# bastienjossen/DDL25Spring

Hardware: AMD Instinct MI355X
Metric: FedAvg rounds/sec + local samples/sec, ResNet-18 CIFAR-10-shape, 8 clients (higher is better)
Workload: dtype fp32; 1 GPU; model=resnet18-cifar10, global_batch=800, parallelism=fedavg-8clients-dp1, clients=8, local_batch=100, local_epochs=1, samples_per_client=6250, client_slots_per_gpu=8, hip_graphs=True, fp32_conv_math=auto

## Files before the change

### csrc/kernels/conv_x6hw.hip

```cpp
#include <cstdlib>

#include "ddl_common.h"
#include "conv_f32_core.h"

namespace {

typedef float f16v __attribute__((ext_vector_type(16)));

constexpr int HW_BK = 64, HW_BC = 32, HW_TP = 128;
constexpr int HW_KS = 136;
constexpr unsigned HW_OOB = 0x80000000u;

struct HWGeo {
  int lgW;
  int SR;
  int NSEG;
  int HR, HCp;
  int CS;
  int ntile;
  int NUX;
  int probe;
};

typedef int hw_rsrc __attribute__((ext_vector_type(4)));
__device__ __forceinline__ hw_rsrc hw_make_rsrc(const void* p, long long bytes) {
  const unsigned long long a = (unsigned long long)p;
  hw_rsrc r;
  r.x = (int)(unsigned)(a & 0xffffffffull);
  r.y = (int)(unsigned)((a >> 32) & 0xffffull);
  r.z = (int)bytes;
  r.w = 0x00020000;
  return r;
}
__device__ __forceinline__ void hw_load(f4v& d, const hw_rsrc& rs, unsigned off) {
  asm volatile("buffer_load_dwordx4 %0, %1, %2, 0 offen" : "=a"(d) : "v"(off), "s"(rs) : "memory");
}

__device__ __forceinline__ void split8(const float (&v)[8], s8v& h, s8v& m, s8v& l) {
  s4v h0, m0, l0, h1, m1, l1;
  split3(make_float4(v[0], v[1], v[2], v[3]), h0, m0, l0);
  split3(make_float4(v[4], v[5], v[6], v[7]), h1, m1, l1);
  h = cat44(h0, h1);
  m = cat44(m0, m1);
  l = cat44(l0, l1);
}

template <int RS, int NUX>
__global__ __launch_bounds__(256, 1) void convx6hw_kernel(ConvF32Args a, HWGeo hg) {
  constexpr int T = RS * RS, PD = (RS - 1) / 2;
  extern __shared__ __attribute__((aligned(16))) char smem[];
  bf16_t* const dyl = (bf16_t*)smem;
  bf16_t* const xl = dyl + 3 * HW_BK * HW_KS;
  const int tid = threadIdx.x, lane = tid & 63, wid = tid >> 6;
  const int OW = 1 << hg.lgW, TR = HW_TP >> hg.lgW;
  const int nct = a.C / HW_BC;
  const int k0 = (blockIdx.x / nct) * HW_BK, c0 = (blockIdx.x % nct) * HW_BC;
  const int split = blockIdx.y, nsplit = gridDim.y, g = blockIdx.z;
  const int per = (hg.ntile + nsplit - 1) / nsplit;
  const int t0 = split * per, t1 = min(hg.ntile, t0 + per);
  const int K = a.K, C = a.C, H = a.H, W = a.W;
  const long long npix = (long long)a.N * H * W;

  const hw_rsrc rD = hw_make_rsrc(a.dy + (long long)g * a.dy_gs, npix * K * 4);
  const hw_rsrc rX = hw_make_rsrc(a.x + (long long)g * a.x_gs, npix * C * 4);

  const int dkc = tid & 15, dpg = tid >> 4;
  const int ncol8 = hg.HCp >> 3;
  const int nxu = 8 * hg.NSEG * hg.HR * ncol8;
  const bool xf = a.in_scale != nullptr;
  float4 xsc[NUX], xsh[NUX];
#pragma unroll
  for (int u = 0; u < NUX; ++u) {
    xsc[u] = make_float4(1.f, 1.f, 1.f, 1.f);
    xsh[u] = make_float4(0.f, 0.f, 0.f, 0.f);
    const int uu = tid + 256 * u;
    if (xf && uu < nxu) {
      const long long cc = (long long)g * C + c0 + 4 * (uu & 7);
      xsc[u] = *(const float4*)(a.in_scale + cc);
      xsh[u] = *(const float4*)(a.in_shift + cc);
    }
  }

  int useg[NUX], uhr[NUX], uxc[NUX], uoff[NUX];
  bool uvalid[NUX];
#pragma unroll
  for (int u = 0; u < NUX; ++u) {
    const int uu = tid + 256 * u, rest = uu >> 3;
    const int xc = rest % ncol8, xrr = rest / ncol8;
    useg[u] = xrr / hg.HR;
    uhr[u] = xrr - useg[u] * hg.HR;
    uxc[u] = xc;
    uoff[u] = 4 * (uu & 7) * hg.CS + xrr * hg.HCp + 8 * xc;
    uvalid[u] = uu < nxu;
  }
  f4v rd[8], rx[NUX][8];
  unsigned xok[NUX];
  auto load_tile = [&](int tile) {
#pragma unroll
    for (int j = 0; j < 8; ++j) {
      const int p = tile * HW_TP + dpg * 8 + j;
      hw_load(rd[j], rD, p < npix ? (unsigned)((p * K + k0 + 4 * dkc) * 4) : HW_OOB);
    }
    const int row0 = tile * TR;
    const int n0 = row0 / a.P, oh0 = row0 - n0 * a.P;
#pragma unroll
    for (int u = 0; u < NUX; ++u) {
      xok[u] = 0;
      const int n = n0 + useg[u];
      const int ih = oh0 + uhr[u] - PD;
#pragma unroll
      for (int j = 0; j < 8; ++j) {
        const int iw = 8 * uxc[u] + j - PD;
        const bool ok = uvalid[u] && n < a.N && (unsigned)ih < (unsigned)H && (unsigned)iw < (unsigned)W;
        xok[u] |= (ok ? 1u : 0u) << j;
        hw_load(rx[u][j], rX, ok ? (unsigned)((((n * H + ih) * W + iw) * C + c0 + 4 * (tid & 7)) * 4) : HW_OOB);
      }
    }
  };
  s8v sd[4][3], sx[NUX][4][3];
  auto hw_wait = [&]() {
    asm volatile("s_waitcnt vmcnt(0)" ::: "memory");
#pragma unroll
    for (int j = 0; j < 8; ++j) asm volatile("" : "+a"(rd[j]));
#pragma unroll
    for (int u = 0; u < NUX; ++u)
#pragma unroll
      for (int j = 0; j < 8; ++j) asm volatile("" : "+a"(rx[u][j]));
  };
  auto split_tile = [&]() {
#pragma unroll
    for (int ch = 0; ch < 4; ++ch) {
      float v[8];
#pragma unroll
      for (int j = 0; j < 8; ++j) v[j] = ch == 0 ? rd[j].x : ch == 1 ? rd[j].y : ch == 2 ? rd[j].z : rd[j].w;
      split8(v, sd[ch][0], sd[ch][1], sd[ch][2]);
    }
  };
  auto write_tile = [&]() {
#pragma unroll
    for (int ch = 0; ch < 4; ++ch) {
      bf16_t* d = dyl + (4 * dkc + ch) * HW_KS + 8 * dpg;
#pragma unroll
      for (int pl = 0; pl < 3; ++pl) *(s8v*)(d + pl * HW_BK * HW_KS) = sd[ch][pl];
    }
#pragma unroll
    for (int u = 0; u < NUX; ++u) {
#pragma unroll
      for (int ch = 0; ch < 4; ++ch) {
        const float sc = ch == 0 ? xsc[u].x : ch == 1 ? xsc[u].y : ch == 2 ? xsc[u].z : xsc[u].w;
        const float sh = ch == 0 ? xsh[u].x : ch == 1 ? xsh[u].y : ch == 2 ? xsh[u].z : xsh[u].w;
        float v[8];
#pragma unroll
        for (int j = 0; j < 8; ++j) {
          float e = ch == 0 ? rx[u][j].x : ch == 1 ? rx[u][j].y : ch == 2 ? rx[u][j].z : rx[u][j].w;
          if (xf && ((xok[u] >> j) & 1u)) {
            e = e * sc + sh;
            if (a.in_relu) e = fmaxf(e, 0.f);
          }
          v[j] = e;
        }
        split8(v, sx[u][ch][0], sx[u][ch][1], sx[u][ch][2]);
      }
    }
#pragma unroll
    for (int u = 0; u < NUX; ++u) {
      if (!uvalid[u]) continue;
#pragma unroll
      for (int ch = 0; ch < 4; ++ch) {
        bf16_t* d = xl + uoff[u] + ch * hg.CS;
#pragma unroll
        for (int pl = 0; pl < 3; ++pl) *(s8v*)(d + pl * HW_BC * hg.CS) = sx[u][ch][pl];
      }
    }
  };

  const int kb = wid >> 1, kh = wid & 1;
  const int arow = (kb * 32 + (lane & 31)) * HW_KS;
  auto xbase = [&](int ks) {
    const int p = 16 * ks + 8 * (lane >> 5);
    const int prow = p >> hg.lgW, pcol = p & (OW - 1);
    const int seg = prow / hg.SR, r = prow - seg * hg.SR;
    return (lane & 31) * hg.CS + (seg * hg.HR + r) * hg.HCp + pcol;
  };
  f16v acc[T];
#pragma unroll
  for (int t = 0; t < T; ++t)
#pragma unroll
    for (int v = 0; v < 16; ++v) acc[t][v] = 0.f;

  if (t0 < t1) {
    if (!(hg.probe & 4)) load_tile(t0);
    for (int tile = t0; tile < t1; ++tile) {
      __syncthreads();
      hw_wait();
      if (!(hg.probe & 1)) {
        split_tile();
        write_tile();
      }
      if (tile + 1 < t1 && !(hg.probe & 4)) load_tile(tile + 1);
      __syncthreads();
      if (hg.probe & 2) continue;
#pragma unroll 1
      for (int ip = 0; ip < 2; ++ip) {
        s8v ah[2], am[2], al[2];
        int xb[2];
#pragma unroll
        for (int j = 0; j < 2; ++j) {
          const int ks = 4 * ip + 2 * j + kh;
          xb[j] = xbase(ks);
          const bf16_t* ap = dyl + arow + 16 * ks + 8 * (lane >> 5);
          ah[j] = *(const s8v*)ap;
          am[j] = *(const s8v*)(ap + HW_BK * HW_KS);
          al[j] = *(const s8v*)(ap + 2 * HW_BK * HW_KS);
        }
#pragma unroll
        for (int r = 0; r < RS; ++r) {
          f16v c[RS];
#pragma unroll
          for (int j = 0; j < 2; ++j) {
            const bf16_t* bp = xl + xb[j] + r * hg.HCp;
            s8v bh[RS], bm[RS], bl[RS];
            const s8v h0 = *(const s8v*)bp, m0 = *(const s8v*)(bp + HW_BC * hg.CS),
                      l0 = *(const s8v*)(bp + 2 * HW_BC * hg.CS);
            bh[0] = h0; bm[0] = m0; bl[0] = l0;
            if constexpr (RS == 3) {
              const s8v h1 = *(const s8v*)(bp + 8), m1 = *(const s8v*)(bp + 8 + HW_BC * hg.CS),
                        l1 = *(const s8v*)(bp + 8 + 2 * HW_BC * hg.CS);
              bh[1] = __builtin_shufflevector(h0, h1, 1, 2, 3, 4, 5, 6, 7, 8);
              bm[1] = __builtin_shufflevector(m0, m1, 1, 2, 3, 4, 5, 6, 7, 8);
              bl[1] = __builtin_shufflevector(l0, l1, 1, 2, 3, 4, 5, 6, 7, 8);
              bh[2] = __builtin_shufflevector(h0, h1, 2, 3, 4, 5, 6, 7, 8, 9);
              bm[2] = __builtin_shufflevector(m0, m1, 2, 3, 4, 5, 6, 7, 8, 9);
              bl[2] = __builtin_shufflevector(l0, l1, 2, 3, 4, 5, 6, 7, 8, 9);
            }
#pragma unroll
            for (int s2 = 0; s2 < RS; ++s2)
              c[s2] = __builtin_amdgcn_mfma_f32_32x32x16_bf16(al[j], bh[s2], j ? c[s2] : (f16v){}, 0, 0, 0);
#pragma unroll
            for (int s2 = 0; s2 < RS; ++s2) c[s2] = __builtin_amdgcn_mfma_f32_32x32x16_bf16(ah[j], bl[s2], c[s2], 0, 0, 0);
#pragma unroll
            for (int s2 = 0; s2 < RS; ++s2) c[s2] = __builtin_amdgcn_mfma_f32_32x32x16_bf16(am[j], bm[s2], c[s2], 0, 0, 0);
#pragma unroll
            for (int s2 = 0; s2 < RS; ++s2) c[s2] = __builtin_amdgcn_mfma_f32_32x32x16_bf16(ah[j], bm[s2], c[s2], 0, 0, 0);
#pragma unroll
            for (int s2 = 0; s2 < RS; ++s2) c[s2] = __builtin_amdgcn_mfma_f32_32x32x16_bf16(am[j], bh[s2], c[s2], 0, 0, 0);
#pragma unroll
            for (int s2 = 0; s2 < RS; ++s2) c[s2] = __builtin_amdgcn_mfma_f32_32x32x16_bf16(ah[j], bh[s2], c[s2], 0, 0, 0);
          }
#pragma unroll
          for (int s2 = 0; s2 < RS; ++s2) {
#pragma unroll
            for (int v = 0; v < 16; ++v) acc[r * RS + s2][v] = acc[r * RS + s2][v] + c[s2][v];
          }
        }
      }
    }
  }

  __syncthreads();
  float* const red = (float*)smem;
  if (kh == 1) {
#pragma unroll
    for (int t = 0; t < T; ++t)
#pragma unroll
      for (int v = 0; v < 16; ++v) red[((kb * T + t) * 16 + v) * 64 + lane] = acc[t][v];
  }
  __syncthreads();
  if (kh == 1) return;
#pragma unroll
  for (int t = 0; t < T; ++t)
#pragma unroll
    for (int v = 0; v < 16; ++v) acc[t][v] = acc[t][v] + red[((kb * T + t) * 16 + v) * 64 + lane];

  const long long qd = (long long)T * C;
  const bool split_store = nsplit > 1;
  float* dst = split_store ? a.partial + ((long long)split * a.G + g) * K * qd : a.out + (long long)g * a.out_gs;
#pragma unroll
  for (int t = 0; t < T; ++t) {
    float old[16];
#pragma unroll
    for (int v = 0; v < 16; ++v) {
      const int k = k0 + kb * 32 + 8 * (v >> 2) + 4 * (lane >> 5) + (v & 3);
      const long long off = (long long)k * qd + (long long)t * C + c0 + (lane & 31);
      old[v] = (!split_store && a.accumulate) ? dst[off] : 0.f;
    }
#pragma unroll
    for (int v = 0; v < 16; ++v) {
      const int k = k0 + kb * 32 + 8 * (v >> 2) + 4 * (lane >> 5) + (v & 3);
      const long long off = (long long)k * qd + (long long)t * C + c0 + (lane & 31);
      dst[off] = split_store ? acc[t][v] : old[v] + a.gscale * acc[t][v];
    }
  }
}

}

static bool hw_geo(const ConvF32Args& a, HWGeo& h, int& rs) {
  if (a.stride != 1 || a.R != a.S || (a.R != 1 && a.R != 3) || a.pad != (a.R - 1) / 2) return false;
  if (a.P != a.H || a.Q != a.W || a.K % HW_BK || a.C % HW_BC) return false;
  const int OW = a.Q, OH = a.P;
  if (OW < 8 || OW > HW_TP || (OW & (OW - 1))) return false;
  rs = a.R;
  int lg = 0;
  while ((1 << lg) < OW) ++lg;
  const int TR = HW_TP / OW;
  int SR;
  if (TR <= OH) {
    if (OH % TR) return false;
    SR = TR;
  } else {
    if (TR % OH) return false;
    SR = OH;
  }
  h.lgW = lg;
  h.SR = SR;
  h.NSEG = TR / SR;
  h.HR = SR + a.R - 1;
  h.HCp = (OW + a.S - 1 + 7) / 8 * 8;
  const int img = h.NSEG * h.HR * h.HCp;
  h.CS = (img - 8 + 127) / 128 * 128 + 8;
  const long long npix = (long long)a.N * a.P * a.Q;
  h.ntile = (int)((npix + HW_TP - 1) / HW_TP);
  const int nxu = 8 * h.NSEG * h.HR * (h.HCp / 8);
  h.NUX = (nxu + 255) / 256;
  if (h.NUX > 2) return false;
  static const int probe = getenv("DDL_HW_PROBE") ? atoi(getenv("DDL_HW_PROBE")) : 0;
  h.probe = probe;
  const long long lim = (1LL << 31) - 64;
  if (npix * a.C * 4 > lim || npix * a.K * 4 > lim) return false;
  return true;
}

static size_t hw_lds(const HWGeo& h, int T) {
  const size_t stage = (size_t)3 * (HW_BK * HW_KS + HW_BC * h.CS) * 2;
  const size_t red = (size_t)2 * T * 16 * 64 * 4;
  return stage > red ? stage : red;
}

extern "C" __attribute__((visibility("default"))) int ddl_x6hw_ok(const ConvF32Args* ap) {
  HWGeo h;
  int rs;
  return hw_geo(*ap, h, rs) && hw_lds(h, rs * rs) <= 160 * 1024 ? 1 : 0;
}

extern "C" __attribute__((visibility("default"))) int ddl_x6hw_tiles(const ConvF32Args* ap) {
  HWGeo h;
  int rs;
  return hw_geo(*ap, h, rs) ? h.ntile : 0;
}

template <int RS, int NUX>
static int launch_hw(const ConvF32Args& a, const HWGeo& h, hipStream_t s) {
  const int split = a.split_k < 1 ? 1 : a.split_k;
  const size_t lds = hw_lds(h, RS * RS);
  static bool attr_set = false;
  if (!attr_set) {
    hipFuncSetAttribute((const void*)convx6hw_kernel<RS, NUX>, hipFuncAttributeMaxDynamicSharedMemorySize,
                        160 * 1024);
    attr_set = true;
  }
  const dim3 grid((unsigned)((a.K / HW_BK) * (a.C / HW_BC)), (unsigned)split, (unsigned)a.G);
  hipLaunchKernelGGL((convx6hw_kernel<RS, NUX>), grid, dim3(256), lds, s, a, h);
  return (int)hipGetLastError();
}

extern "C" __attribute__((visibility("default"))) int ddl_x6hw(const ConvF32Args* ap, hipStream_t s) {
  const ConvF32Args& a = *ap;
  HWGeo h;
  int rs;
  if (a.G < 1 || a.N < 1 || !hw_geo(a, h, rs) || hw_lds(h, rs * rs) > 160 * 1024) return (int)hipErrorInvalidValue;
  const int split = a.split_k < 1 ? 1 : a.split_k;
  if (split > 1) {
    const long long need = (long long)split * a.G * a.K * a.R * a.S * a.C;
    if (!a.partial || need > a.partial_cap) return (int)hipErrorInvalidValue;
  }
  int e;
  if (rs == 3) e = h.NUX == 1 ? launch_hw<3, 1>(a, h, s) : launch_hw<3, 2>(a, h, s);
  else e = h.NUX == 1 ? launch_hw<1, 1>(a, h, s) : launch_hw<1, 2>(a, h, s);
  return e;
}
```

### ddl25spring_amd/ops/functional_f32.py

```python
from __future__ import annotations

import ctypes
import math
import os

import torch

from . import _lib
from . import workspace as ws
from ._lib import check, ptr, stream

F_FWD, F_DGRAD, F_WGRAD = 0, 1, 2
WS_CAP = 1 << 26
_WS: dict = {}
TARGET_WG = int(os.environ.get("DDL_F32_TARGET_WG", "640"))


def is_f32(t) -> bool:
    return t is not None and t.is_cuda and t.dtype == torch.float32


class SlotStats:
    __slots__ = ("t", "rows")

# ... 377 lines not shown
    def __exit__(self, *exc):
        _PRESPLIT[0] = self._prev
        if self._pending is not None:
            torch.cuda.current_stream().wait_event(self._pending)
            self._pending = None
        if self.state == "record" and self.keys and not torch.cuda.is_current_stream_capturing() \
                and exc[0] is None:
            self._build()
        return False

    def _build(self):
        lib = _lib.kernels()
        if lib.ddl_x6_split_desc_size() != ctypes.sizeof(_SplitDesc):
            raise RuntimeError("ABI mismatch for SplitDesc")
        dev = torch.device("cuda", torch.cuda.current_device())
        vol = [k[2] * k[3] * k[4] * k[5] for k in self.keys]
        nhead = len(self.keys)
        if PRESPLIT_SIDE[0] and len(self.keys) > 1:
            nhead, acc = 1, vol[0]
            while nhead < len(self.keys) and acc + vol[nhead] <= PRESPLIT_HEAD_FRAC * sum(vol):
                acc += vol[nhead]
                nhead += 1
        self.tail = set(self.keys[nhead:])
        self.tables = []
        for part in (self.keys[:nhead], self.keys[nhead:]):
            if not part:
                continue
            descs = (_SplitDesc * len(part))()
            blk = 0
            for i, key in enumerate(part):
                w, layout, G, K, T, C, w_gs = key
                buf = torch.empty(G, K * T * C * 6, dtype=torch.uint8, device=dev)
                self.bufs[key] = buf
                nblk = max(1, min(1024, -(-G * K * T * C // 16 // 256)))
                d = descs[i]
                d.w, d.out, d.w_gs, d.o_gs = w, buf.data_ptr(), w_gs, buf.stride(0)
                d.G, d.K, d.T, d.C, d.layout, d.blk0, d.nblk = G, K, T, C, layout, blk, nblk
                blk += nblk
            raw = torch.frombuffer(bytearray(bytes(descs)), dtype=torch.uint8)
            self.tables.append((raw.to(dev), len(part), blk))
        self.state = "ready"


def _store_identity(owner):
    store = getattr(owner, "store", None)
    data = getattr(store, "data", None)
    if data is None:
        return None
    return data.data_ptr(), data.numel(), id(data.untyped_storage())


def presplit_scope(owner) -> "PresplitScope | contextlib.nullcontext":
    sig = _store_identity(owner)
    sc = getattr(owner, "_f32_presplit", None)
    if sc is None or getattr(owner, "_f32_presplit_sig", None) != sig:
        sc = PresplitScope()
        owner._f32_presplit = sc
        owner._f32_presplit_sig = sig
    return sc


def _slots(a, mode: int, geom) -> int:
    cfg, _ = plan(mode, geom)
    if uses_halo(mode, geom):
        return int(_lib.kernels().ddl_x6h_slots(ctypes.byref(a), mode))
    return int(_lib.kernels().ddl_convf32_slots(ctypes.byref(a), mode, _cfg(cfg)))


def slot_rows(mode: int, geom) -> int:
    cfg, _ = plan(mode, geom)
    bq = ((_cfg(cfg) >> 8) & 0xFF) * 16
    if uses_halo(mode, geom) and geom.Q & (geom.Q - 1):
        return bq // (1 << (geom.Q - 1).bit_length()) * geom.Q
    return bq


def _xform(in_bn):
    if in_bn is None:
        return {}
    sc, sh = in_bn
    assert sc.is_contiguous() and sh.is_contiguous()
    return dict(in_scale=ptr(sc), in_shift=ptr(sh), in_relu=1)


def conv_fwd(x, w, geom, bias=None, relu=False, stats=None, out=None, residual=None, in_bn=None, split_k=0):
    y = out if out is not None else torch.empty(geom.G, geom.N, geom.P, geom.Q, geom.K, dtype=torch.float32,
                                                device=x.device)
    if residual is not None and (residual.stride(0) != y.stride(0) or not residual.is_contiguous()):
        residual = residual.contiguous()
    geom = _launch_geom(geom, "f")
    a = _args(geom, x=ptr(x), w=ptr(w), out=ptr(y), bias=ptr(bias), residual=ptr(residual),
              x_gs=_gs(x), w_gs=_gs(w), out_gs=_gs(y), bias_gs=_gs(bias), relu=int(bool(relu)), **_xform(in_bn))
    if stats is not None:
        st = torch.empty(geom.G, _slots(a, F_FWD, geom), 2, geom.K, dtype=torch.float32, device=x.device)
        a.stats = ptr(st)
        if isinstance(stats, SlotStats):
            stats.t = st
            stats.rows = slot_rows(F_FWD, geom)
        else:
            raise TypeError("fp32 conv statistics go to a SlotStats (Fn.stats_buffer(..., like=x))")
    _launch(a, F_FWD, geom, x.device, split_k)
    return y


def conv_dgrad(dy, w, geom, residual=None, mask=None, out=None, bn=None, mask_bn=None, residual_sub=1,
               split_k=0, dy_bn=None, dy_bn_out=None):
    dx = out if out is not None else torch.empty(geom.G, geom.N, geom.H, geom.W, geom.C, dtype=torch.float32,
                                                 device=dy.device)
    if residual_sub == 1:
        geom = _launch_geom(geom, "d")
    kw = {}
    if dy_bn is not None:
        xb, coef = dy_bn
        assert xb.is_contiguous() and coef.is_contiguous() and xb.shape == dy.shape and dy.is_contiguous()
        if uses_halo(F_DGRAD, geom) and split_k == 0:
            kw.update(dyb_x=ptr(xb), dyb_coef=ptr(coef), dyb_out=ptr(dy_bn_out))
        else:
            dy = coef_apply(dy, xb, coef, out=dy_bn_out)
    if residual is not None and residual_sub == 2 and geom.H & 1 and uses_halo(F_DGRAD, geom) \
            and (split_k or plan(F_DGRAD, geom)[1]) <= 1:
        full = torch.zeros_like(dx)
        full[:, :, ::2, ::2] = residual
        residual, residual_sub = full, 1
    if residual is not None:
        if residual_sub == 2:
            want = (geom.G, geom.N, (geom.H + 1) // 2, (geom.W + 1) // 2, geom.C)
            assert tuple(residual.shape) == want, (tuple(residual.shape), want)
            residual = residual.contiguous()
            kw.update(res_sub=2, res_gs=residual.stride(0))
        elif residual.stride(0) != dx.stride(0) or not residual.is_contiguous():
            residual = residual.contiguous()
    if mask is not None and (mask.stride(0) != dx.stride(0) or not mask.is_contiguous()):
        mask = mask.contiguous()
    if bn is not None:
        x, mean, rstd = bn
        assert x.is_contiguous() and x.stride(0) == dx.stride(0) and mean.is_contiguous() and rstd.is_contiguous()
        kw.update(bn_x=ptr(x), bn_mean=ptr(mean), bn_rstd=ptr(rstd))
        if mask_bn is not None:
            sc, sh = mask_bn
            assert sc.is_contiguous() and sh.is_contiguous() and sc.numel() == geom.G * geom.C
            kw.update(mask_scale=ptr(sc), mask_shift=ptr(sh))
    a = _args(geom, w=ptr(w), dy=ptr(dy), out=ptr(dx), residual=ptr(residual), mask=ptr(mask),
              w_gs=_gs(w), dy_gs=_gs(dy), out_gs=_gs(dx), **kw)
    part = None
    if bn is not None:
        part = torch.empty(geom.G, _slots(a, F_DGRAD, geom), 2, geom.C, dtype=torch.float32, device=dy.device)
        a.stats = ptr(part)
    _launch(a, F_DGRAD, geom, dy.device, split_k)
    return dx if bn is None else (dx, part)


HALO_WGRAD = [os.environ.get("DDL_F32_HALO_WGRAD", "1") != "0"]
HW_MIN_W = int(os.environ.get("DDL_F32_HW_MIN_W", "16"))
HW_TARGET_WG = int(os.environ.get("DDL_F32_HW_TARGET_WG", "256"))


def uses_halo_wgrad(geom) -> bool:
    a = _args(geom)
    return HALO_WGRAD[0] and _MATH[0] != "mfma32" and geom.W >= HW_MIN_W \
        and bool(_lib.kernels().ddl_x6hw_ok(ctypes.byref(a)))


def _halo_wgrad(a, geom, device, split_k: int, ws_role: str) -> bool:
    if not (HALO_WGRAD[0] and _MATH[0] != "mfma32") or geom.W < HW_MIN_W \
            or not _lib.kernels().ddl_x6hw_ok(ctypes.byref(a)):
        return False
    lib = _lib.kernels()
    ntile = int(lib.ddl_x6hw_tiles(ctypes.byref(a)))
    base = (geom.K // 64) * (geom.C // 32) * geom.G
    split = split_k or 1
    if not split_k and TARGET_WG != 1:
        _tuned(F_WGRAD, geom)
        p = _TUNED.get(f"x6hw:wgrad:{geom.G},{geom.N},{geom.H},{geom.W},{geom.C},{geom.K},{geom.R},{geom.S},"
                       f"{geom.stride},{geom.pad}")
        if p is not None:
            split_k = split = int(p[0])
    if not split_k:
        target = min(HW_TARGET_WG, TARGET_WG)
        while base * split < target and ntile >= split * 2 * 3 and split < 128:
            split *= 2
    n = geom.K * geom.R * geom.S * geom.C
    if split > 1:
        buf = workspace(device, ws_role)
        while split > 1 and split * geom.G * n > buf.numel():
            split //= 2
        if split > 1:
            a.partial, a.partial_cap = buf.data_ptr(), buf.numel()
    a.split_k = split
    check(lib.ddl_x6hw(ctypes.byref(a), stream()), "conv_wgrad_f32_halo")
    if split > 1:
        check(lib.ddl_convf32_wgrad_reduce(a.partial, a.out, a.out_gs, geom.G, n, split, a.accumulate, a.gscale,
                                           stream()), "conv_wgrad_f32_halo_reduce")
    return True


def conv_wgrad(dy, x, geom, dw, accumulate=True, gscale=1.0, in_bn=None, split_k=0, ws_role="main"):
    if not accumulate and gscale != 1.0:
        raise ValueError("a scaled WGRAD must accumulate (it adds into the master weights)")
    geom = _launch_geom(geom, "w")
    a = _args(geom, x=ptr(x), dy=ptr(dy), out=ptr(dw), x_gs=_gs(x), dy_gs=_gs(dy), out_gs=_gs(dw),
              accumulate=int(bool(accumulate)), gscale=float(gscale), **_xform(in_bn))
    if (F_WGRAD, geom) not in _OVERRIDE and _halo_wgrad(a, geom, dy.device, split_k, ws_role):
        return dw
    _launch(a, F_WGRAD, geom, dy.device, split_k, ws_role)
    return dw


def _bnf_args(stats, gamma, beta, running_mean, running_var, count, eps, momentum, training, outs, G, C,
              tile_rows=0):
    a = _lib.BNFArgs()
    a.tile_rows = int(tile_rows)
    a.stats, a.gamma, a.beta = ptr(stats), ptr(gamma), ptr(beta)
    a.running_mean, a.running_var = ptr(running_mean), ptr(running_var)
    a.scale, a.shift, a.mean, a.rstd = (ptr(outs[i]) for i in range(4))
    a.gs_param = _gs(gamma) if gamma is not None else _gs(beta)
    a.gs_buf = _gs(running_mean)
    a.G, a.C, a.count = G, C, int(count)
    a.eps, a.momentum, a.training = float(eps), float(momentum), int(training)
    a.stripes = stats.shape[1] if stats is not None else 0
    return a


def bn_finalize_many(items, eps=1e-5, momentum=0.1, training=True):
    dev = items[0][1].device if items[0][1] is not None else items[0][3].device
    args, outs = [], []
    for stats, gamma, beta, rm, rv, count, G, C in items:
        t = stats.t if isinstance(stats, SlotStats) else stats
        rows = stats.rows if isinstance(stats, SlotStats) else 0
        if training:
            assert t is not None and t.is_contiguous(), "fp32 BN statistics missing (conv not run?)"
        o = torch.empty(4, G, C, dtype=torch.float32, device=dev)
        args.append(_bnf_args(t if training else None, gamma, beta, rm, rv, count, eps, momentum, training, o, G, C,
                              rows))
        outs.append(o)
    b = ctypes.byref(args[1]) if len(args) > 1 else None
    check(_lib.kernels().ddl_bnf_finalize(ctypes.byref(args[0]), b, stream()), "bn_finalize_f32")
    return [(o[0], o[1], o[2], o[3]) for o in outs]


def bn_apply(x, scale, shift, r=None, rscale=None, rshift=None, act=0, out=None):
    assert x.is_contiguous() and (r is None or r.is_contiguous())
    y = out if out is not None else torch.empty_like(x)
    G, C = x.shape[0], x.shape[-1]
    check(_lib.kernels().ddl_bnf_apply(ptr(x), ptr(scale), ptr(shift), ptr(r), ptr(rscale), ptr(rshift), ptr(y),
                                       x[0].numel(), C, G, act, stream()), "bn_apply_f32")
    return y


def reduce_slots(M: int, C: int, G: int) -> int:
    return int(_lib.kernels().ddl_bnf_reduce_slots(int(M), int(C), int(G)))


def bn_bwd_reduce_part(dy, ymask, x, mean, rstd):
    G, C = x.shape[0], x.shape[-1]
    M = x[0].numel() // C
    part = torch.empty(G, reduce_slots(M, C, G), 2, C, dtype=torch.float32, device=x.device)
    check(_lib.kernels().ddl_bnf_reduce(ptr(dy), ptr(ymask), ptr(x), ptr(mean), ptr(rstd), ptr(part), M, C, G,
                                        stream()), "bn_bwd_reduce_f32")
    return part


def bn_stats(x):
    G, C = x.shape[0], x.shape[-1]
    M = x[0].numel() // C
    st = SlotStats()
    st.t = torch.empty(G, reduce_slots(M, C, G), 2, C, dtype=torch.float32, device=x.device)
    check(_lib.kernels().ddl_bnf_stats(ptr(x), ptr(st.t), M, C, G, stream()), "bn_stats_f32")
    return st


def _bwd_args(x, mean, rstd, gamma, dgamma, dbeta, part, dx, fold_slots: int = 0, coef=None):
    G, C = x.shape[0], x.shape[-1]
    t = _lib.BNFBwdArgs()
    if coef is None:
        coef = ws.scratch_uninit((G, 3, C), x.device)
    gs = _gs(gamma) if gamma is not None else 0
    if dgamma is not None or dbeta is not None:
        gd = _gs(dgamma) if dgamma is not None else _gs(dbeta)
        assert gamma is None or gd == gs, "gamma and its gradient must share the group stride"
        gs = gd
    t.x, t.mean, t.rstd, t.gamma = ptr(x), ptr(mean), ptr(rstd), ptr(gamma)
    t.dgamma, t.dbeta, t.part, t.coef, t.dx, t.gs_param = ptr(dgamma), ptr(dbeta), ptr(part), ptr(coef), ptr(dx), gs
    t.slots = part.shape[1] if part is not None else 0
    S = max(fold_slots, t.slots)
    fws = None
    if FOLD2[0] and S > 0:
        fws = torch.empty(int(_lib.kernels().ddl_bnf_fold_ws(S, C, G)), dtype=torch.float64, device=x.device)
        t.fold_ws = fws.data_ptr()
        if FOLD1L[0] and x.is_cuda:
            t.tickets = _fold_tickets(x.device, int(_lib.kernels().ddl_bnf_fold_tickets(C, G)))
    t._keep = (coef, fws)
    return t


FOLD2 = [os.environ.get("DDL_F32_FOLD2", "1") != "0"]
FOLD1L = [os.environ.get("DDL_F32_FOLD1L", "1") != "0"]
_TICKETS: dict = {}


TICKETS_N = 1 << 16


def _dev_key(device) -> str:
    d = torch.device(device)
    return f"cuda:{d.index if d.index is not None else torch.cuda.current_device()}"


def _fold_tickets(device, n: int) -> int:
    key = _dev_key(device)
    buf = _TICKETS.get(key)
    if buf is None:
        if torch.cuda.is_current_stream_capturing():
            raise RuntimeError("fp32 BN fold counters first requested inside a graph capture: run one eager "
                               "step (or functional_f32.ensure_workspace) before capturing")
        buf = torch.zeros(TICKETS_N, dtype=torch.int32, device=device)
        _TICKETS[key] = buf
    if n > buf.numel():
        raise ValueError(f"BN fold needs {n} counters (> {buf.numel()})")
    return buf.data_ptr()


def fold_tickets_clean() -> bool:
    torch.cuda.synchronize()
    return all(int(b.abs().sum().item()) == 0 for b in _TICKETS.values())


def bn_backward(dy, ymask, x, mean, rstd, gamma, dgamma=None, dbeta=None, emit_dym=False, part=None):
    G, C = x.shape[0], x.shape[-1]
    M = x[0].numel() // C
    assert dy.is_contiguous() and x.is_contiguous()
    do_reduce = part is None
    if do_reduce:
# ... 115 lines not shown
```

Before: 38310 samples/s.

## Warp-specialize halo wgrad kernel with double-buffered LDS staging waves

Restructures the halo weight-gradient conv kernel into 512 threads, with four producer waves that load, split to bf16x3 and stage tiles into a double-buffered LDS region. Four consumer waves run the MFMA loops, so global loads and splitting overlap with matrix math instead of alternating with it. The pixel tile is halved to 64, and the split granularity is now counted in tile pairs. It also adds a W=4 variant, which the Python side only uses for small widths when a tuned entry exists. In exchange it doubles LDS usage, holds two register tile sets in the producers, and changes how split-K is sized.

Result: faster. 39270 samples/s (median of 6 runs) (+2.5%).

```diff
diff --git a/csrc/kernels/conv_x6hw.hip b/csrc/kernels/conv_x6hw.hip
--- a/csrc/kernels/conv_x6hw.hip
+++ b/csrc/kernels/conv_x6hw.hip
@@ -7,8 +7,10 @@
 
 typedef float f16v __attribute__((ext_vector_type(16)));
 
-constexpr int HW_BK = 64, HW_BC = 32, HW_TP = 128;
-constexpr int HW_KS = 136;
+constexpr int HW_BK = 64, HW_BC = 32, HW_TP = 64;
+constexpr int HW_KS = 72;
+constexpr int HW_NT = 512;
+constexpr size_t HW_LDS_MAX = 160 * 1024;
 constexpr unsigned HW_OOB = 0x80000000u;
 
 struct HWGeo {
@@ -18,7 +20,6 @@
   int HR, HCp;
   int CS;
   int ntile;
-  int NUX;
   int probe;
 };
 
@@ -33,7 +34,7 @@
   return r;
 }
 __device__ __forceinline__ void hw_load(f4v& d, const hw_rsrc& rs, unsigned off) {
-  asm volatile("buffer_load_dwordx4 %0, %1, %2, 0 offen" : "=a"(d) : "v"(off), "s"(rs) : "memory");
+  asm volatile("buffer_load_dwordx4 %0, %1, %2, 0 offen" : "=v"(d) : "v"(off), "s"(rs) : "memory");
 }
 
 __device__ __forceinline__ void split8(const float (&v)[8], s8v& h, s8v& m, s8v& l) {
@@ -45,18 +46,35 @@
   l = cat44(l0, l1);
 }
 
-template <int RS, int NUX>
-__global__ __launch_bounds__(256, 1) void convx6hw_kernel(ConvF32Args a, HWGeo hg) {
+template <bool W4>
+__device__ __forceinline__ s8v hw_win(const s8v& c0, const s8v& c1, int s) {
+  if constexpr (W4) {
+    if (s == 0) return __builtin_shufflevector(c0, c1, 0, 1, 2, 3, 8, 9, 10, 11);
+    if (s == 1) return __builtin_shufflevector(c0, c1, 1, 2, 3, 4, 9, 10, 11, 12);
+    return __builtin_shufflevector(c0, c1, 2, 3, 4, 5, 10, 11, 12, 13);
+  } else {
+    if (s == 0) return c0;
+    if (s == 1) return __builtin_shufflevector(c0, c1, 1, 2, 3, 4, 5, 6, 7, 8);
+    return __builtin_shufflevector(c0, c1, 2, 3, 4, 5, 6, 7, 8, 9);
+  }
+}
+
+template <int RS, bool W4>
+__global__ __launch_bounds__(HW_NT) void convx6hw_kernel(ConvF32Args a, HWGeo hg) {
   constexpr int T = RS * RS, PD = (RS - 1) / 2;
   extern __shared__ __attribute__((aligned(16))) char smem[];
+  const int stg = 3 * (HW_BK * HW_KS + HW_BC * hg.CS);
   bf16_t* const dyl = (bf16_t*)smem;
   bf16_t* const xl = dyl + 3 * HW_BK * HW_KS;
-  const int tid = threadIdx.x, lane = tid & 63, wid = tid >> 6;
+  const int tid = threadIdx.x, lane = tid & 63;
+  const int wid = __builtin_amdgcn_readfirstlane(tid >> 6);
+  const bool stager = wid < 4;
+  const int ptid = tid & 255;
   const int OW = 1 << hg.lgW, TR = HW_TP >> hg.lgW;
   const int nct = a.C / HW_BC;
   const int k0 = (blockIdx.x / nct) * HW_BK, c0 = (blockIdx.x % nct) * HW_BC;
   const int split = blockIdx.y, nsplit = gridDim.y, g = blockIdx.z;
-  const int per = (hg.ntile + nsplit - 1) / nsplit;
+  const int per = 2 * (((hg.ntile + 1) / 2 + nsplit - 1) / nsplit);
   const int t0 = split * per, t1 = min(hg.ntile, t0 + per);
   const int K = a.K, C = a.C, H = a.H, W = a.W;
   const long long npix = (long long)a.N * H * W;
@@ -64,196 +82,187 @@
   const hw_rsrc rD = hw_make_rsrc(a.dy + (long long)g * a.dy_gs, npix * K * 4);
   const hw_rsrc rX = hw_make_rsrc(a.x + (long long)g * a.x_gs, npix * C * 4);
 
-  const int dkc = tid & 15, dpg = tid >> 4;
-  const int ncol8 = hg.HCp >> 3;
-  const int nxu = 8 * hg.NSEG * hg.HR * ncol8;
-  const bool xf = a.in_scale != nullptr;
-  float4 xsc[NUX], xsh[NUX];
-#pragma unroll
-  for (int u = 0; u < NUX; ++u) {
-    xsc[u] = make_float4(1.f, 1.f, 1.f, 1.f);
-    xsh[u] = make_float4(0.f, 0.f, 0.f, 0.f);
-    const int uu = tid + 256 * u;
-    if (xf && uu < nxu) {
-      const long long cc = (long long)g * C + c0 + 4 * (uu & 7);
-      xsc[u] = *(const float4*)(a.in_scale + cc);
-      xsh[u] = *(const float4*)(a.in_shift + cc);
-    }
-  }
-
-  int useg[NUX], uhr[NUX], uxc[NUX], uoff[NUX];
-  bool uvalid[NUX];
-#pragma unroll
-  for (int u = 0; u < NUX; ++u) {
-    const int uu = tid + 256 * u, rest = uu >> 3;
-    const int xc = rest % ncol8, xrr = rest / ncol8;
-    useg[u] = xrr / hg.HR;
-    uhr[u] = xrr - useg[u] * hg.HR;
-    uxc[u] = xc;
-    uoff[u] = 4 * (uu & 7) * hg.CS + xrr * hg.HCp + 8 * xc;
-    uvalid[u] = uu < nxu;
-  }
-  f4v rd[8], rx[NUX][8];
-  unsigned xok[NUX];
-  auto load_tile = [&](int tile) {
-#pragma unroll
-    for (int j = 0; j < 8; ++j) {
-      const int p = tile * HW_TP + dpg * 8 + j;
-      hw_load(rd[j], rD, p < npix ? (unsigned)((p * K + k0 + 4 * dkc) * 4) : HW_OOB);
-    }
-    const int row0 = tile * TR;
-    const int n0 = row0 / a.P, oh0 = row0 - n0 * a.P;
-#pragma unroll
-    for (int u = 0; u < NUX; ++u) {
-      xok[u] = 0;
-      const int n = n0 + useg[u];
-      const int ih = oh0 + uhr[u] - PD;
+  const int nt = t1 - t0;
+
+  if (stager) {
+    const int dkc = (ptid & 3) | (((ptid >> 4) & 3) << 2), dpg = ((ptid >> 2) & 3) | (((ptid >> 6) & 3) << 2);
+    const int ucg = (ptid & 1) | (((ptid >> 3) & 3) << 1), urest = ((ptid >> 1) & 3) | (((ptid >> 5) & 7) << 2);
+    const int ncol8 = hg.HCp >> 3;
+    const bool uvalid = urest < hg.NSEG * hg.HR * ncol8;
+    const int uxc = urest % ncol8, xrr = urest / ncol8;
+    const int useg = xrr / hg.HR, uhr = xrr - useg * hg.HR;
+    const int uoff = 4 * ucg * hg.CS + xrr * hg.HCp + 8 * uxc;
+    const bool xf = a.in_scale != nullptr;
+    float4 xsc = make_float4(1.f, 1.f, 1.f, 1.f), xsh = make_float4(0.f, 0.f, 0.f, 0.f);
+    if (xf && uvalid) {
+      const long long cc = (long long)g * C + c0 + 4 * ucg;
+      xsc = *(const float4*)(a.in_scale + cc);
+      xsh = *(const float4*)(a.in_shift + cc);
+    }
+
+    struct Regs {
+      f4v d[4], x[8];
+      unsigned ok;
+    };
+    constexpr int NLD = 12;
+    auto load_tile = [&](int tile, Regs& q) {
+      if (hg.probe & 4) return;
+#pragma unroll
+      for (int j = 0; j < 4; ++j) {
+        const long long p = (long long)tile * HW_TP + dpg * 4 + j;
+        hw_load(q.d[j], rD, p < npix ? (unsigned)(((int)p * K + k0 + 4 * dkc) * 4) : HW_OOB);
+      }
+      const int row0 = tile * TR;
+      const int n0 = row0 / a.P, oh0 = row0 - n0 * a.P;
+      const int n = n0 + useg;
+      const int ih = oh0 + uhr - PD;
+      q.ok = 0;
 #pragma unroll
       for (int j = 0; j < 8; ++j) {
-        const int iw = 8 * uxc[u] + j - PD;
-        const bool ok = uvalid[u] && n < a.N && (unsigned)ih < (unsigned)H && (unsigned)iw < (unsigned)W;
-        xok[u] |= (ok ? 1u : 0u) << j;
-        hw_load(rx[u][j], rX, ok ? (unsigned)((((n * H + ih) * W + iw) * C + c0 + 4 * (tid & 7)) * 4) : HW_OOB);
-      }
-    }
-  };
-  s8v sd[4][3], sx[NUX][4][3];
-  auto hw_wait = [&]() {
-    asm volatile("s_waitcnt vmcnt(0)" ::: "memory");
-#pragma unroll
-    for (int j = 0; j < 8; ++j) asm volatile("" : "+a"(rd[j]));
-#pragma unroll
-    for (int u = 0; u < NUX; ++u)
-#pragma unroll
-      for (int j = 0; j < 8; ++j) asm volatile("" : "+a"(rx[u][j]));
-  };
-  auto split_tile = [&]() {
-#pragma unroll
-    for (int ch = 0; ch < 4; ++ch) {
-      float v[8];
-#pragma unroll
-      for (int j = 0; j < 8; ++j) v[j] = ch == 0 ? rd[j].x : ch == 1 ? rd[j].y : ch == 2 ? rd[j].z : rd[j].w;
-      split8(v, sd[ch][0], sd[ch][1], sd[ch][2]);
-    }
-  };
-  auto write_tile = [&]() {
-#pragma unroll
-    for (int ch = 0; ch < 4; ++ch) {
-      bf16_t* d = dyl + (4 * dkc + ch) * HW_KS + 8 * dpg;
-#pragma unroll
-      for (int pl = 0; pl < 3; ++pl) *(s8v*)(d + pl * HW_BK * HW_KS) = sd[ch][pl];
-    }
-#pragma unroll
-    for (int u = 0; u < NUX; ++u) {
+        const int iw = 8 * uxc + j - PD;
+        const bool ok = uvalid && n < a.N && (unsigned)ih < (unsigned)H && (unsigned)iw < (unsigned)W;
+        q.ok |= (ok ? 1u : 0u) << j;
+        hw_load(q.x[j], rX, ok ? (unsigned)((((n * H + ih) * W + iw) * C + c0 + 4 * ucg) * 4) : HW_OOB);
+      }
+    };
+    auto hw_wait = [&](Regs& q) {
+      asm volatile("s_waitcnt vmcnt(%0)" ::"n"(NLD) : "memory");
+#pragma unroll
+      for (int j = 0; j < 4; ++j) asm volatile("" : "+v"(q.d[j]));
+#pragma unroll
+      for (int j = 0; j < 8; ++j) asm volatile("" : "+v"(q.x[j]));
+    };
+    auto write_tile = [&](int b, const Regs& q) {
+      if (hg.probe & 1) return;
+      bf16_t* const dys = dyl + b * stg;
+      bf16_t* const xs = xl + b * stg;
 #pragma unroll
       for (int ch = 0; ch < 4; ++ch) {
-        const float sc = ch == 0 ? xsc[u].x : ch == 1 ? xsc[u].y : ch == 2 ? xsc[u].z : xsc[u].w;
-        const float sh = ch == 0 ? xsh[u].x : ch == 1 ? xsh[u].y : ch == 2 ? xsh[u].z : xsh[u].w;
+        float4 v;
+        v.x = ch == 0 ? q.d[0].x : ch == 1 ? q.d[0].y : ch == 2 ? q.d[0].z : q.d[0].w;
+        v.y = ch == 0 ? q.d[1].x : ch == 1 ? q.d[1].y : ch == 2 ? q.d[1].z : q.d[1].w;
+        v.z = ch == 0 ? q.d[2].x : ch == 1 ? q.d[2].y : ch == 2 ? q.d[2].z : q.d[2].w;
+        v.w = ch == 0 ? q.d[3].x : ch == 1 ? q.d[3].y : ch == 2 ? q.d[3].z : q.d[3].w;
+        s4v h, m, l;
+        split3(v, h, m, l);
+        bf16_t* d = dys + (4 * dkc + ch) * HW_KS + 4 * dpg;
+        *(s4v*)d = h;
+        *(s4v*)(d + HW_BK * HW_KS) = m;
+        *(s4v*)(d + 2 * HW_BK * HW_KS) = l;
+      }
+      if (!uvalid) return;
+#pragma unroll
+      for (int ch = 0; ch < 4; ++ch) {
+        const float sc = ch == 0 ? xsc.x : ch == 1 ? xsc.y : ch == 2 ? xsc.z : xsc.w;
+        const float sh = ch == 0 ? xsh.x : ch == 1 ? xsh.y : ch == 2 ? xsh.z : xsh.w;
         float v[8];
 #pragma unroll
         for (int j = 0; j < 8; ++j) {
-          float e = ch == 0 ? rx[u][j].x : ch == 1 ? rx[u][j].y : ch == 2 ? rx[u][j].z : rx[u][j].w;
-          if (xf && ((xok[u] >> j) & 1u)) {
+          float e = ch == 0 ? q.x[j].x : ch == 1 ? q.x[j].y : ch == 2 ? q.x[j].z : q.x[j].w;
+          if (xf && ((q.ok >> j) & 1u)) {
             e = e * sc + sh;
             if (a.in_relu) e = fmaxf(e, 0.f);
           }
           v[j] = e;
         }
-        split8(v, sx[u][ch][0], sx[u][ch][1], sx[u][ch][2]);
-      }
-    }
-#pragma unroll
-    for (int u = 0; u < NUX; ++u) {
-      if (!uvalid[u]) continue;
-#pragma unroll
-      for (int ch = 0; ch < 4; ++ch) {
-        bf16_t* d = xl + uoff[u] + ch * hg.CS;
-#pragma unroll
-        for (int pl = 0; pl < 3; ++pl) *(s8v*)(d + pl * HW_BC * hg.CS) = sx[u][ch][pl];
-      }
-    }
-  };
-
-  const int kb = wid >> 1, kh = wid & 1;
-  const int arow = (kb * 32 + (lane & 31)) * HW_KS;
-  auto xbase = [&](int ks) {
+        s8v h, m, l;
+        split8(v, h, m, l);
+        bf16_t* d = xs + uoff + ch * hg.CS;
+        *(s8v*)d = h;
+        *(s8v*)(d + HW_BC * hg.CS) = m;
+        *(s8v*)(d + 2 * HW_BC * hg.CS) = l;
+      }
+    };
+    if (nt > 0) {
+      Regs qa, qb;
+      load_tile(t0, qa);
+      load_tile(t0 + 1, qb);
+      hw_wait(qa);
+      write_tile(0, qa);
+      load_tile(t0 + 2, qa);
+      __syncthreads();
+      auto step = [&](int i, Regs& q) {
+        if (i + 1 < nt) {
+          hw_wait(q);
+          write_tile((i + 1) & 1, q);
+          load_tile(t0 + i + 3, q);
+        }
+        __syncthreads();
+      };
+      for (int i = 0; i < nt; i += 2) {
+        step(i, qb);
+        if (i + 1 < nt) step(i + 1, qa);
+      }
+    }
+    __syncthreads();
+    __syncthreads();
+    return;
+  }
+
+  const int kb = (wid >> 1) & 1, kh = wid & 1;
+  int ao[2], xb[2];
+#pragma unroll
+  for (int j = 0; j < 2; ++j) {
+    const int ks = 2 * j + kh;
     const int p = 16 * ks + 8 * (lane >> 5);
     const int prow = p >> hg.lgW, pcol = p & (OW - 1);
     const int seg = prow / hg.SR, r = prow - seg * hg.SR;
-    return (lane & 31) * hg.CS + (seg * hg.HR + r) * hg.HCp + pcol;
+    ao[j] = (kb * 32 + (lane & 31)) * HW_KS + p;
+    xb[j] = (lane & 31) * hg.CS + (seg * hg.HR + r) * hg.HCp + pcol;
+  }
+  const int c1o = W4 ? hg.HCp : 8;
+  f16v acc[T];
+#pragma unroll
+  for (int t = 0; t < T; ++t)
+#pragma unroll
+    for (int v = 0; v < 16; ++v) acc[t][v] = 0.f;
+
+  auto compute_tile = [&](int b) {
+    const bf16_t* const dys = dyl + b * stg;
+    const bf16_t* const xs = xl + b * stg;
+    s8v ah[2], am[2], al[2];
+#pragma unroll
+    for (int j = 0; j < 2; ++j) {
+      const bf16_t* ap = dys + ao[j];
+      ah[j] = *(const s8v*)ap;
+      am[j] = *(const s8v*)(ap + HW_BK * HW_KS);
+      al[j] = *(const s8v*)(ap + 2 * HW_BK * HW_KS);
+    }
+#pragma unroll
+    for (int r = 0; r < RS; ++r) {
+#pragma unroll
+      for (int s2 = 0; s2 < RS; ++s2) {
+        f16v c;
+#pragma unroll
+        for (int j = 0; j < 2; ++j) {
+          const bf16_t* bp = xs + xb[j] + r * hg.HCp;
+          const s8v h0 = *(const s8v*)bp, m0 = *(const s8v*)(bp + HW_BC * hg.CS),
+                    l0 = *(const s8v*)(bp + 2 * HW_BC * hg.CS);
+          s8v h1 = h0, m1 = m0, l1 = l0;
+          if (W4 || s2 > 0) {
+            h1 = *(const s8v*)(bp + c1o);
+            m1 = *(const s8v*)(bp + c1o + HW_BC * hg.CS);
+            l1 = *(const s8v*)(bp + c1o + 2 * HW_BC * hg.CS);
+          }
+          const s8v bh = hw_win<W4>(h0, h1, s2), bm = hw_win<W4>(m0, m1, s2), bl = hw_win<W4>(l0, l1, s2);
+          c = __builtin_amdgcn_mfma_f32_32x32x16_bf16(al[j], bh, j ? c : (f16v){}, 0, 0, 0);
+          c = __builtin_amdgcn_mfma_f32_32x32x16_bf16(ah[j], bl, c, 0, 0, 0);
+          c = __builtin_amdgcn_mfma_f32_32x32x16_bf16(am[j], bm, c, 0, 0, 0);
+          c = __builtin_amdgcn_mfma_f32_32x32x16_bf16(ah[j], bm, c, 0, 0, 0);
+          c = __builtin_amdgcn_mfma_f32_32x32x16_bf16(am[j], bh, c, 0, 0, 0);
+          c = __builtin_amdgcn_mfma_f32_32x32x16_bf16(ah[j], bh, c, 0, 0, 0);
+        }
+#pragma unroll
+        for (int v = 0; v < 16; ++v) acc[r * RS + s2][v] = acc[r * RS + s2][v] + c[v];
+      }
+    }
   };
-  f16v acc[T];
-#pragma unroll
-  for (int t = 0; t < T; ++t)
-#pragma unroll
-    for (int v = 0; v < 16; ++v) acc[t][v] = 0.f;
-
-  if (t0 < t1) {
-    if (!(hg.probe & 4)) load_tile(t0);
-    for (int tile = t0; tile < t1; ++tile) {
+
+  if (nt > 0) {
+    __syncthreads();
+    for (int i = 0; i < nt; ++i) {
+      if (!(hg.probe & 2)) compute_tile(i & 1);
       __syncthreads();
-      hw_wait();
-      if (!(hg.probe & 1)) {
-        split_tile();
-        write_tile();
-      }
-      if (tile + 1 < t1 && !(hg.probe & 4)) load_tile(tile + 1);
-      __syncthreads();
-      if (hg.probe & 2) continue;
-#pragma unroll 1
-      for (int ip = 0; ip < 2; ++ip) {
-        s8v ah[2], am[2], al[2];
-        int xb[2];
-#pragma unroll
-        for (int j = 0; j < 2; ++j) {
-          const int ks = 4 * ip + 2 * j + kh;
-          xb[j] = xbase(ks);
-          const bf16_t* ap = dyl + arow + 16 * ks + 8 * (lane >> 5);
-          ah[j] = *(const s8v*)ap;
-          am[j] = *(const s8v*)(ap + HW_BK * HW_KS);
-          al[j] = *(const s8v*)(ap + 2 * HW_BK * HW_KS);
-        }
-#pragma unroll
-        for (int r = 0; r < RS; ++r) {
-          f16v c[RS];
-#pragma unroll
-          for (int j = 0; j < 2; ++j) {
-            const bf16_t* bp = xl + xb[j] + r * hg.HCp;
-            s8v bh[RS], bm[RS], bl[RS];
-            const s8v h0 = *(const s8v*)bp, m0 = *(const s8v*)(bp + HW_BC * hg.CS),
-                      l0 = *(const s8v*)(bp + 2 * HW_BC * hg.CS);
-            bh[0] = h0; bm[0] = m0; bl[0] = l0;
-            if constexpr (RS == 3) {
-              const s8v h1 = *(const s8v*)(bp + 8), m1 = *(const s8v*)(bp + 8 + HW_BC * hg.CS),
-                        l1 = *(const s8v*)(bp + 8 + 2 * HW_BC * hg.CS);
-              bh[1] = __builtin_shufflevector(h0, h1, 1, 2, 3, 4, 5, 6, 7, 8);
-              bm[1] = __builtin_shufflevector(m0, m1, 1, 2, 3, 4, 5, 6, 7, 8);
-              bl[1] = __builtin_shufflevector(l0, l1, 1, 2, 3, 4, 5, 6, 7, 8);
-              bh[2] = __builtin_shufflevector(h0, h1, 2, 3, 4, 5, 6, 7, 8, 9);
-              bm[2] = __builtin_shufflevector(m0, m1, 2, 3, 4, 5, 6, 7, 8, 9);
-              bl[2] = __builtin_shufflevector(l0, l1, 2, 3, 4, 5, 6, 7, 8, 9);
-            }
-#pragma unroll
-            for (int s2 = 0; s2 < RS; ++s2)
-              c[s2] = __builtin_amdgcn_mfma_f32_32x32x16_bf16(al[j], bh[s2], j ? c[s2] : (f16v){}, 0, 0, 0);
-#pragma unroll
-            for (int s2 = 0; s2 < RS; ++s2) c[s2] = __builtin_amdgcn_mfma_f32_32x32x16_bf16(ah[j], bl[s2], c[s2], 0, 0, 0);
-#pragma unroll
-            for (int s2 = 0; s2 < RS; ++s2) c[s2] = __builtin_amdgcn_mfma_f32_32x32x16_bf16(am[j], bm[s2], c[s2], 0, 0, 0);
-#pragma unroll
-            for (int s2 = 0; s2 < RS; ++s2) c[s2] = __builtin_amdgcn_mfma_f32_32x32x16_bf16(ah[j], bm[s2], c[s2], 0, 0, 0);
-#pragma unroll
-            for (int s2 = 0; s2 < RS; ++s2) c[s2] = __builtin_amdgcn_mfma_f32_32x32x16_bf16(am[j], bh[s2], c[s2], 0, 0, 0);
-#pragma unroll
-            for (int s2 = 0; s2 < RS; ++s2) c[s2] = __builtin_amdgcn_mfma_f32_32x32x16_bf16(ah[j], bh[s2], c[s2], 0, 0, 0);
-          }
-#pragma unroll
-          for (int s2 = 0; s2 < RS; ++s2) {
-#pragma unroll
-            for (int v = 0; v < 16; ++v) acc[r * RS + s2][v] = acc[r * RS + s2][v] + c[s2][v];
-          }
-        }
-      }
     }
   }
 
@@ -267,28 +276,41 @@
   }
   __syncthreads();
   if (kh == 1) return;
-#pragma unroll
-  for (int t = 0; t < T; ++t)
+  auto tap_sum = [&](int t) {
+    __builtin_amdgcn_sched_barrier(0);
 #pragma unroll
     for (int v = 0; v < 16; ++v) acc[t][v] = acc[t][v] + red[((kb * T + t) * 16 + v) * 64 + lane];
-
-  const long long qd = (long long)T * C;
+  };
+
+  const int qd = T * C;
   const bool split_store = nsplit > 1;
-  float* dst = split_store ? a.partial + ((long long)split * a.G + g) * K * qd : a.out + (long long)g * a.out_gs;
-#pragma unroll
-  for (int t = 0; t < T; ++t) {
-    float old[16];
-#pragma unroll
-    for (int v = 0; v < 16; ++v) {
-      const int k = k0 + kb * 32 + 8 * (v >> 2) + 4 * (lane >> 5) + (v & 3);
-      const long long off = (long long)k * qd + (long long)t * C + c0 + (lane & 31);
-      old[v] = (!split_store && a.accumulate) ? dst[off] : 0.f;
-    }
-#pragma unroll
-    for (int v = 0; v < 16; ++v) {
-      const int k = k0 + kb * 32 + 8 * (v >> 2) + 4 * (lane >> 5) + (v & 3);
-      const long long off = (long long)k * qd + (long long)t * C + c0 + (lane & 31);
-      dst[off] = split_store ? acc[t][v] : old[v] + a.gscale * acc[t][v];
+  float* const dst = (split_store ? a.partial + ((long long)split * a.G + g) * K * qd : a.out + (long long)g * a.out_gs) +
+                     (long long)(k0 + kb * 32) * qd + c0;
+  const unsigned loff = (unsigned)((4 * (lane >> 5) * qd + (lane & 31)) * 4);
+  auto eptr = [&](int t, int v) { return (float*)((char*)(dst + (8 * (v >> 2) + (v & 3)) * qd + t * C) + loff); };
+  if (split_store) {
+#pragma unroll
+    for (int t = 0; t < T; ++t) {
+      tap_sum(t);
+#pragma unroll
+      for (int v = 0; v < 16; ++v) *eptr(t, v) = acc[t][v];
+    }
+  } else if (a.accumulate) {
+#pragma unroll
+    for (int t = 0; t < T; ++t) {
+      tap_sum(t);
+      float old[16];
+#pragma unroll
+      for (int v = 0; v < 16; ++v) old[v] = *eptr(t, v);
+#pragma unroll
+      for (int v = 0; v < 16; ++v) *eptr(t, v) = old[v] + a.gscale * acc[t][v];
+    }
+  } else {
+#pragma unroll
+    for (int t = 0; t < T; ++t) {
+      tap_sum(t);
+#pragma unroll
+      for (int v = 0; v < 16; ++v) *eptr(t, v) = 0.f + a.gscale * acc[t][v];
     }
   }
 }
@@ -299,7 +321,7 @@
   if (a.stride != 1 || a.R != a.S || (a.R != 1 && a.R != 3) || a.pad != (a.R - 1) / 2) return false;
   if (a.P != a.H || a.Q != a.W || a.K % HW_BK || a.C % HW_BC) return false;
   const int OW = a.Q, OH = a.P;
-  if (OW < 8 || OW > HW_TP || (OW & (OW - 1))) return false;
+  if (OW < 4 || OW > HW_TP || (OW & (OW - 1))) return false;
   rs = a.R;
   int lg = 0;
   while ((1 << lg) < OW) ++lg;
@@ -312,6 +334,7 @@
     if (TR % OH) return false;
     SR = OH;
   }
+  if (OW == 4 && (SR & 1)) return false;
   h.lgW = lg;
   h.SR = SR;
   h.NSEG = TR / SR;
@@ -322,45 +345,45 @@
   const long long npix = (long long)a.N * a.P * a.Q;
   h.ntile = (int)((npix + HW_TP - 1) / HW_TP);
   const int nxu = 8 * h.NSEG * h.HR * (h.HCp / 8);
-  h.NUX = (nxu + 255) / 256;
-  if (h.NUX > 2) return false;
+  if (nxu > 256) return false;
   static const int probe = getenv("DDL_HW_PROBE") ? atoi(getenv("DDL_HW_PROBE")) : 0;
   h.probe = probe;
   const long long lim = (1LL << 31) - 64;
   if (npix * a.C * 4 > lim || npix * a.K * 4 > lim) return false;
+  if ((long long)a.K * a.R * a.S * a.C * 4 > lim) return false;
   return true;
 }
 
 static size_t hw_lds(const HWGeo& h, int T) {
-  const size_t stage = (size_t)3 * (HW_BK * HW_KS + HW_BC * h.CS) * 2;
+  const size_t stages = (size_t)2 * 3 * (HW_BK * HW_KS + HW_BC * h.CS) * 2;
   const size_t red = (size_t)2 * T * 16 * 64 * 4;
-  return stage > red ? stage : red;
+  return stages > red ? stages : red;
 }
 
 extern "C" __attribute__((visibility("default"))) int ddl_x6hw_ok(const ConvF32Args* ap) {
   HWGeo h;
   int rs;
-  return hw_geo(*ap, h, rs) && hw_lds(h, rs * rs) <= 160 * 1024 ? 1 : 0;
+  return hw_geo(*ap, h, rs) && hw_lds(h, rs * rs) <= HW_LDS_MAX ? 1 : 0;
 }
 
 extern "C" __attribute__((visibility("default"))) int ddl_x6hw_tiles(const ConvF32Args* ap) {
   HWGeo h;
   int rs;
-  return hw_geo(*ap, h, rs) ? h.ntile : 0;
-}
-
-template <int RS, int NUX>
+  return hw_geo(*ap, h, rs) ? (h.ntile + 1) / 2 : 0;
+}
+
+template <int RS, bool W4>
 static int launch_hw(const ConvF32Args& a, const HWGeo& h, hipStream_t s) {
   const int split = a.split_k < 1 ? 1 : a.split_k;
   const size_t lds = hw_lds(h, RS * RS);
   static bool attr_set = false;
   if (!attr_set) {
-    hipFuncSetAttribute((const void*)convx6hw_kernel<RS, NUX>, hipFuncAttributeMaxDynamicSharedMemorySize,
-                        160 * 1024);
+    hipFuncSetAttribute((const void*)convx6hw_kernel<RS, W4>, hipFuncAttributeMaxDynamicSharedMemorySize,
+                        (int)HW_LDS_MAX);
     attr_set = true;
   }
   const dim3 grid((unsigned)((a.K / HW_BK) * (a.C / HW_BC)), (unsigned)split, (unsigned)a.G);
-  hipLaunchKernelGGL((convx6hw_kernel<RS, NUX>), grid, dim3(256), lds, s, a, h);
+  hipLaunchKernelGGL((convx6hw_kernel<RS, W4>), grid, dim3(HW_NT), lds, s, a, h);
   return (int)hipGetLastError();
 }
 
@@ -368,14 +391,12 @@
   const ConvF32Args& a = *ap;
   HWGeo h;
   int rs;
-  if (a.G < 1 || a.N < 1 || !hw_geo(a, h, rs) || hw_lds(h, rs * rs) > 160 * 1024) return (int)hipErrorInvalidValue;
+  if (a.G < 1 || a.N < 1 || !hw_geo(a, h, rs) || hw_lds(h, rs * rs) > HW_LDS_MAX) return (int)hipErrorInvalidValue;
   const int split = a.split_k < 1 ? 1 : a.split_k;
   if (split > 1) {
     const long long need = (long long)split * a.G * a.K * a.R * a.S * a.C;
     if (!a.partial || need > a.partial_cap) return (int)hipErrorInvalidValue;
   }
-  int e;
-  if (rs == 3) e = h.NUX == 1 ? launch_hw<3, 1>(a, h, s) : launch_hw<3, 2>(a, h, s);
-  else e = h.NUX == 1 ? launch_hw<1, 1>(a, h, s) : launch_hw<1, 2>(a, h, s);
-  return e;
-}
+  if (rs == 3) return h.lgW == 2 ? launch_hw<3, true>(a, h, s) : launch_hw<3, false>(a, h, s);
+  return h.lgW == 2 ? launch_hw<1, true>(a, h, s) : launch_hw<1, false>(a, h, s);
+}
diff --git a/ddl25spring_amd/ops/functional_f32.py b/ddl25spring_amd/ops/functional_f32.py
--- a/ddl25spring_amd/ops/functional_f32.py
+++ b/ddl25spring_amd/ops/functional_f32.py
@@ -553,32 +553,43 @@
 
 HALO_WGRAD = [os.environ.get("DDL_F32_HALO_WGRAD", "1") != "0"]
 HW_MIN_W = int(os.environ.get("DDL_F32_HW_MIN_W", "16"))
+HW_MIN_W_PINNED = "DDL_F32_HW_MIN_W" in os.environ
 HW_TARGET_WG = int(os.environ.get("DDL_F32_HW_TARGET_WG", "256"))
+HW_MIN_TILES = 3
+
+
+def _hw_entry(geom):
+    _tuned(F_WGRAD, geom)
+    return _TUNED.get(f"x6hw:wgrad:{geom.G},{geom.N},{geom.H},{geom.W},{geom.C},{geom.K},{geom.R},{geom.S},"
+                      f"{geom.stride},{geom.pad}")
+
+
+def _hw_takes(a, geom) -> bool:
+    if not (HALO_WGRAD[0] and _MATH[0] != "mfma32"):
+        return False
+    if geom.W < HW_MIN_W and (HW_MIN_W_PINNED or _hw_entry(geom) is None):
+        return False
+    return bool(_lib.kernels().ddl_x6hw_ok(ctypes.byref(a)))
 
 
 def uses_halo_wgrad(geom) -> bool:
-    a = _args(geom)
-    return HALO_WGRAD[0] and _MATH[0] != "mfma32" and geom.W >= HW_MIN_W \
-        and bool(_lib.kernels().ddl_x6hw_ok(ctypes.byref(a)))
+    return _hw_takes(_args(geom), geom)
 
 
 def _halo_wgrad(a, geom, device, split_k: int, ws_role: str) -> bool:
-    if not (HALO_WGRAD[0] and _MATH[0] != "mfma32") or geom.W < HW_MIN_W \
-            or not _lib.kernels().ddl_x6hw_ok(ctypes.byref(a)):
+    if not _hw_takes(a, geom):
         return False
     lib = _lib.kernels()
     ntile = int(lib.ddl_x6hw_tiles(ctypes.byref(a)))
     base = (geom.K // 64) * (geom.C // 32) * geom.G
     split = split_k or 1
     if not split_k and TARGET_WG != 1:
-        _tuned(F_WGRAD, geom)
-        p = _TUNED.get(f"x6hw:wgrad:{geom.G},{geom.N},{geom.H},{geom.W},{geom.C},{geom.K},{geom.R},{geom.S},"
-                       f"{geom.stride},{geom.pad}")
+        p = _hw_entry(geom)
         if p is not None:
             split_k = split = int(p[0])
     if not split_k:
         target = min(HW_TARGET_WG, TARGET_WG)
-        while base * split < target and ntile >= split * 2 * 3 and split < 128:
+        while base * split < target and ntile >= split * 2 * HW_MIN_TILES and split < 128:
             split *= 2
     n = geom.K * geom.R * geom.S * geom.C
     if split > 1:
```
